# Hi-FT/ERD

Hardware: AMD Instinct MI355X
Metric: images/sec GFL-R50 40+40 incre step @1333x800 (higher is better)
Workload: dtype f32; 1 GPU; gfl_r50_fpn first_40_incre_last_40 ERD (BASELINE configs[1]), 1333x800 padded to 800x1344, fp32, procedural weights; batch_per_gpu=4, global_batch=4, parallelism=dp1

## Files before the change

### erd_amd/_lib.py

```python
from __future__ import annotations

import ctypes as C
import os

_HERE = os.path.dirname(os.path.abspath(__file__))
LIB_PATH = os.environ.get("ERD_HIP_LIB") or os.path.join(_HERE, "lib", "liberd_hip.so")

ERD_MAX_SEG = 5
ERD_MAX_TAPS = 9
ERD_SQNORM_PARTS = 1024

c_float_p = C.c_void_p
i64 = C.c_int64
i32 = C.c_int
f32 = C.c_float


class ConvSeg(C.Structure):
    _fields_ = [("inp", C.c_void_p), ("out", C.c_void_p), ("res", C.c_void_p), ("alpha", C.c_void_p),
                ("mask", C.c_void_p), ("N", i32), ("IH", i32), ("IW", i32), ("GH", i32), ("GW", i32), ("OH", i32), ("OW", i32),
                ("in_nstride", i64), ("out_nstride", i64), ("res_nstride", i64),
                ("tap0", i32), ("ntaps", i32), ("oy", i32), ("ox", i32)]


# ... 34 lines not shown


class Levels(C.Structure):
    _fields_ = [("nseg", i32), ("off", i64 * ERD_MAX_SEG), ("cnt", i64 * ERD_MAX_SEG)]


P = C.c_void_p
_SIGNATURES = {
    "erd_set_cu_reserve": [i32],
    "erd_usable_cus": [],
    "erd_conv_igemm": [C.POINTER(ConvDesc), P],
    "erd_conv_igemm_ws_bytes": [i32],
    "erd_to_bf16": [P, P, i64, P],
    "erd_split3": [P, P, i64, P],
    "erd_conv_thin_enable": [i32],
    "erd_conv_thin_ok": [C.POINTER(ConvDesc)],
    "erd_weight_transpose_x3": [P, P, P, i32, i32, i32, i32, P],
    "erd_wino_weights_elems": [i32, i32],
    "erd_wino_weights": [P, P, i32, i32, i32, P],
    "erd_wino_conv3x3": [P, i32, P, i32, i32, P, P, i32, P, i32, P, P],
    "erd_wino_weights_x3_elems": [i32, i32],
    "erd_wino_weights_x3": [P, P, i32, i32, i32, P],
    "erd_wino_conv3x3_x3": [P, i32, P, i32, i32, P, P, i32, P, i32, P, P],
    "erd_wino_x3_couts_per_item": [P, i32, i32],
    "erd_wino_conv3x3_x3_gn": [P, i32, P, i32, i32, P, P, i32, P, P, C.c_size_t, P],
    "erd_wino_gn_finalize": [P, i32, i32, P, P, f32, P],
    "erd_wino_x3_gn_ws_bytes": [P, i32, i32],
    "erd_conv_wgrad": [C.POINTER(WgradDesc), P],
    "erd_wgrad_row3_slices": [C.POINTER(WgradDesc)],
    "erd_wgrad_reduce": [P, i32, i32, i32, P, P, P, i32, P, P],
    "erd_wgrad_reduce_rows": [P, i32, i32, i32, i32, P, i32, P],
    "erd_weight_transpose": [P, P, P, i32, i32, i32, i32, P],
    "erd_weight_transpose_bf16": [P, P, P, i32, i32, i32, i32, P],
    "erd_stem_conv7x7_bn_relu": [P, P, P, P, P, i32, i32, i32, P],
    "erd_maxpool3x3s2": [P, P, i32, i32, i32, i32, i32, P],
    "erd_bn_fold": [P, P, P, P, f32, P, P, i64, P],
    "erd_bn_fold_batch": [P, i32, i32, P],
    "erd_weight_prep_blocks": [i32, i32, i32, i32],
    "erd_weight_prep_batch": [P, i32, i32, P],
    "erd_relu_bwd_colsum": [P, P, P, i64, i32, i64, i64, P, i32, i32, P],
    "erd_bn_dgamma": [P, P, i32, P, P, f32, P, P, i32, i32, P],
    "erd_gn_relu_fwd": [P, P, P, P, P, P, i32, i64, i32, i32, C.POINTER(Levels), f32, i32, P],
    "erd_gn_relu_apply": [P, P, P, P, P, i32, i64, i32, i32, C.POINTER(Levels), i32, P],
    "erd_gn_relu_bwd": [P, P, P, P, P, P, P, P, P, i32, i64, i32, i32, C.POINTER(Levels), i32, P],
    "erd_upsample2x_add": [P, P, i32, i32, i32, i32, i32, i32, i64, i64, i32, P],
    "erd_upsample2x_add_bwd": [P, P, i32, i32, i32, i32, i32, i32, i64, i64, i32, P],
# ... 90 lines not shown
```

### erd_amd/csrc/winograd.hip

```cpp
#include "erd_common.h"
#include <type_traits>
#include <stdlib.h>
#include <algorithm>

namespace {

typedef float f32x4 __attribute__((ext_vector_type(4)));
typedef unsigned int u32x4 __attribute__((ext_vector_type(4)));
constexpr unsigned OOBV = 0x80000000u;

__device__ __forceinline__ float4 buf_load16_s(__amdgpu_buffer_rsrc_t r, unsigned voff, unsigned soff) {
    const u32x4 v = __builtin_amdgcn_raw_buffer_load_b128(r, voff, soff, 0);
    return make_float4(__uint_as_float(v.x), __uint_as_float(v.y), __uint_as_float(v.z), __uint_as_float(v.w));
}

constexpr int KS = 16;
constexpr int BN = 64;
constexpr int BNP = 128;
constexpr int RCS = 6;
#ifndef ERD_WINO_NCH
#define ERD_WINO_NCH 4
#endif
constexpr int NCH = ERD_WINO_NCH;
constexpr int MAXPIX = 64 * NCH;
constexpr int RAW_LDS_F4 = MAXPIX * RCS;
constexpr int V_F4 = 16 * 32 * (KS / 4);
constexpr int MAXREG = 16;

__device__ __forceinline__ float4 f4add(float4 a, float4 b) { return make_float4(a.x + b.x, a.y + b.y, a.z + b.z, a.w + b.w); }
__device__ __forceinline__ float4 f4sub(float4 a, float4 b) { return make_float4(a.x - b.x, a.y - b.y, a.z - b.z, a.w - b.w); }
__device__ __forceinline__ int vswz2(int row, int c) { return c ^ ((0 - (row >> 2)) & 3); }

#ifdef ERD_WINO_TRACE
__device__ unsigned long long g_wino_trace[256 * 8];
__device__ unsigned long long g_wino_trace_p[256 * 16];
#define ERD_T0(v) const unsigned long long v = __builtin_amdgcn_s_memtime()
#define ERD_TACC(acc, v) acc += __builtin_amdgcn_s_memtime() - v
#else
#define ERD_T0(v)
#define ERD_TACC(acc, v)
#endif

__global__ __launch_bounds__(256) void wino_weight_kernel(const float* __restrict__ w, float* __restrict__ U, int Cout,
                                                           int Cin, int flip) {
    const int cop = (Cout + 15) / 16 * 16;
    const int64_t idx = blockIdx.x * 256ll + threadIdx.x;
    if (idx >= (int64_t)cop * Cin) return;
    const int co = (int)(idx / Cin), ci = (int)(idx % Cin);
    float g[3][3];
#pragma unroll
// ... 951 lines not shown
            };
            for (int g = 0;;) {
                if (g >= slices_total) break;
                iter(P0{}, P1{});
                if (++g >= slices_total) break;
                iter(P1{}, P0{});
                ++g;
            }
        };
        if (t_half == 0) run(std::integral_constant<int, 0>{});
        else run(std::integral_constant<int, 1>{});
#ifdef ERD_WINO_TRACE
        if (wave == 0 && lane == 0 && blockIdx.x < 256) {
            g_wino_trace[blockIdx.x * 8 + 4] = __builtin_amdgcn_s_memtime() - t_begin;
            g_wino_trace[blockIdx.x * 8 + 5] = t_bar;
            g_wino_trace[blockIdx.x * 8 + 6] = t_ent;
            g_wino_trace[blockIdx.x * 8 + 7] = t_wait;
        }
#endif
    }
}

constexpr int HPIX = 208;

__global__ __launch_bounds__(512, 2) void wino_x3p_kernel(const WinoDesc p) {
    extern __shared__ __attribute__((aligned(16))) char smem[];
    constexpr unsigned RAWB = HPIX * RCS * 16, VOFF = 2 * RAWB, VB = VX_B, XOFF = VOFF + 2 * VB;
    float* sh_ss = reinterpret_cast<float*>(smem + XOFF);
    int* sh_item = reinterpret_cast<int*>(sh_ss + 4 * 2 * BNP);
    float* sh_gn = reinterpret_cast<float*>(sh_item + 4);
    char* const sm = smem;

    const int tid = threadIdx.x;
    const int Cin = p.Cin;
    const int nks = Cin / KS;
    const int nitems = p.nitems;
    const int ncb32 = (p.Cout + 31) / 32;
    int cur_item = blockIdx.x;


    const int wave = __builtin_amdgcn_readfirstlane(tid >> 6), lane = tid & 63;
    const int item0 = blockIdx.x;
    if (item0 >= nitems) return;

    const int li = lane & 31, h = lane >> 5;
    const int ri = wave & 3, cp = wave >> 2;
    const int t_chunk = tid & 3, t_tile = (tid >> 2) & 31;
    const int t_row = __builtin_amdgcn_readfirstlane(tid >> 7);
    const int rowA = t_row == 0 ? 0 : (t_row == 2 ? 2 : 1), rowB = t_row == 2 ? 1 : (t_row == 3 ? 3 : 2);

    const __amdgpu_buffer_rsrc_t rs_U = __builtin_amdgcn_make_buffer_rsrc(
        const_cast<void*>(p.U3), 0, (int)((size_t)16 * 3 * ncb32 * nks * 1024), 0x00020000);
    const unsigned u_lane = (unsigned)lane * 16u;
    const unsigned per_xl_b = (unsigned)ncb32 * (unsigned)nks * 1024u;
    const unsigned pos0_b = (unsigned)(ri * 4 * 3) * per_xl_b;
    const unsigned cb_b = (unsigned)nks * 1024u;
    const unsigned v_lane = (unsigned)(ri * 4 * 3 * 1024 + h * 512 + ((li ^ (h * 8)) * 16));
    WinoItem cur = wino_decode<BNP>(p, item0);
    int k_item = 0;
    unsigned u_item = (unsigned)__builtin_amdgcn_readfirstlane(((cur.cout0 >> 5) + 2 * cp) * nks * 1024);
    f32x16 acc[8];
    u32x4 ub[4][3];
    bf16x8 vf[2][3];
    auto load_u = [&](const int u, const unsigned soff) {
#pragma unroll
        for (int l = 0; l < 3; ++l)
            ub[u & 3][l] = __builtin_amdgcn_raw_buffer_load_b128(rs_U, u_lane, pos0_b + (unsigned)((u >> 1) * 3 + l) * per_xl_b + soff + (u & 1) * cb_b, 0);
    };

    WinoItem la = cur;
    int la_ks = 0, k_la = 0;
    unsigned la_soff = 0;
    bool la_valid = true;
    unsigned roff[2];
    float4 rv[2];
    __amdgpu_buffer_rsrc_t rs_in = __builtin_amdgcn_make_buffer_rsrc(const_cast<float*>(p.seg[0].in), 0, 0, 0x00020000);
    unsigned rdA = 0, rdB = 0, nrdA = 0, nrdB = 0;
    int tr_left = 0;
    auto item_geometry = [&](const WinoItem& it, unsigned (&ro)[2], unsigned& gA, unsigned& gB, __amdgpu_buffer_rsrc_t& rs) {
        const WinoSeg& sg = p.seg[it.s];
        rs = __builtin_amdgcn_make_buffer_rsrc(const_cast<float*>(sg.in), 0, (int)((long long)sg.N * sg.in_nstride * 4), 0x00020000);
        const int lbw = it.lbw, bw = 1 << lbw, bh = 32 >> lbw;
        const int pc_n = 2 * bw + 2, npix = (2 * bh + 2) * pc_n;
        const int recip = (65536 + pc_n - 1) / pc_n;
        const unsigned base_n = (unsigned)(it.n * sg.in_nstride);
#pragma unroll
        for (int i = 0; i < 2; ++i) {
            const int idx = tid + 512 * i;
            const int chunk = idx & 3, pix = idx >> 2;
            const int pr = (pix * recip) >> 16, pc = pix - pr * pc_n;
            const int iy = it.y0 - 1 + pr, ix = it.x0 - 1 + pc;
            ro[i] = OOBV;
            if (pix < npix && (unsigned)iy < (unsigned)sg.H && (unsigned)ix < (unsigned)sg.W)
                ro[i] = (base_n + (unsigned)((iy * sg.W + ix) * Cin + chunk * 4)) * 4u;
        }
        const int t_ty = t_tile >> lbw, t_tx = t_tile & (bw - 1);
        gA = (unsigned)((((2 * t_ty + rowA) * pc_n + 2 * t_tx) * RCS + t_chunk) * 16);
        gB = (unsigned)((((2 * t_ty + rowB) * pc_n + 2 * t_tx) * RCS + t_chunk) * 16);
    };
    struct Pending { float sc, sh; int claim, k; };
    auto request_item_data = [&](Pending& pe) {
        if (tid < BNP) {
            const int co = la.cout0 + tid;
            pe.sc = (p.scale && co < p.Cout) ? p.scale[co] : 1.f;
            pe.sh = (p.shift && co < p.Cout) ? p.shift[co] : 0.f;
        }
        if (tid == BNP) pe.claim = wino_claim(p, k_la);
        pe.k = k_la;
    };
    auto flush_pending = [&](const Pending& pe) {
        if (pe.k >= 0) {
            if (tid < BNP) {
                float* ss = sh_ss + (pe.k & 3) * (2 * BNP);
                ss[tid] = pe.sc;
                ss[BNP + tid] = pe.sh;
            }
            if (tid == BNP) sh_item[(pe.k + 1) & 1] = pe.claim;
        }
    };
    auto issue_next = [&](float4* dst) {
        if (la_valid) {
#pragma unroll
            for (int i = 0; i < 2; ++i) dst[i] = buf_load16_s(rs_in, roff[i], la_soff);
            la_soff += KS * 4;
            ++la_ks;
        }
    };
    auto advance_item = [&](Pending& pe) {
        if (la_valid && la_ks == nks) {
            const int nx = __builtin_amdgcn_readfirstlane(sh_item[(k_la + 1) & 1]);
            if (nx < nitems) {
                la = wino_decode<BNP>(p, nx);
                item_geometry(la, roff, nrdA, nrdB, rs_in);
                la_ks = 0;
                la_soff = 0;
                ++k_la;
                request_item_data(pe);
            } else la_valid = false;
        }
    };
    const bool st1_ok = (tid >> 2) + 128 < HPIX;
    auto store_raw = [&](const float4* src, const unsigned par) {
        int t = tid;
        asm volatile("" : "+v"(t));
        const unsigned st_base = (unsigned)(((t >> 2) * RCS + (t & 3)) * 16);
        *reinterpret_cast<float4*>(sm + par * RAWB + st_base) = src[0];
        if (st1_ok) *reinterpret_cast<float4*>(sm + par * RAWB + st_base + 128 * RCS * 16) = src[1];
    };
    float4 pd[2][4];
    auto transform_read = [&](const unsigned rpar) {
        const char* rA = sm + rpar * RAWB + rdA;
        const char* rB = sm + rpar * RAWB + rdB;
#pragma unroll
        for (int c = 0; c < 4; ++c) {
            pd[0][c] = *reinterpret_cast<const float4*>(rA + c * (RCS * 16));
            pd[1][c] = *reinterpret_cast<const float4*>(rB + c * (RCS * 16));
        }
        if (--tr_left == 0) {
            rdA = nrdA;
            rdB = nrdB;
            tr_left = nks;
        }
    };
    auto v_write_base = [&]() -> unsigned {
        int t = tid;
        asm volatile("" : "+v"(t));
        const int c = t & 3, tl = (t >> 2) & 31;
        return VOFF + (unsigned)(t_row * 4 * 3072 + (c >> 1) * 512 + ((tl ^ ((c >> 1) * 8)) * 16) + (c & 1) * 8);
    };
    auto row_pass = [&](float4 (&R)[4]) __attribute__((always_inline)) {
        if (t_row == 1) {
#pragma unroll
            for (int c = 0; c < 4; ++c) R[c] = f4add(pd[0][c], pd[1][c]);
        } else {
#pragma unroll
            for (int c = 0; c < 4; ++c) R[c] = f4sub(pd[0][c], pd[1][c]);
        }
    };
    unsigned long long t_d1 = 0, t_d2 = 0, t_d3 = 0, t_out = 0; (void)t_d1; (void)t_d2; (void)t_d3; (void)t_out;
    auto data_phase = [&](const unsigned par, const unsigned u_tail) __attribute__((always_inline)) {
        const unsigned npar = par ^ 1u;
        ERD_T0(ta);
        transform_read(npar);
        __builtin_amdgcn_sched_barrier(0);
// ... 168 lines not shown
                        float* cpt = p.colsum + (p.colsum_copies > 1 ? (blockIdx.x & (p.colsum_copies - 1)) * p.Cout : 0) + co0;
                        atomicAdd(cpt + 0, cs[gq].x); atomicAdd(cpt + 1, cs[gq].y); atomicAdd(cpt + 2, cs[gq].z); atomicAdd(cpt + 3, cs[gq].w);
                    }
                }
            }
            __syncthreads();
        }
        if (p.gn_part && tid < 32) {
            const float t = ((sh_gn[tid] + sh_gn[32 + tid]) + sh_gn[64 + tid]) + sh_gn[96 + tid];
            p.gn_part[(int64_t)cur_item * 32 + tid] = t;
        }
    };

    {
        float4 rvb[2];
#pragma unroll
        for (int i = 0; i < 2; ++i) { rv[i] = make_float4(0.f, 0.f, 0.f, 0.f); rvb[i] = rv[i]; }
        item_geometry(la, roff, nrdA, nrdB, rs_in);
        Pending pe;
        pe.sc = 1.f; pe.sh = 0.f; pe.claim = 0; pe.k = -1;
        request_item_data(pe);
        rdA = nrdA;
        rdB = nrdB;
        tr_left = nks;
        flush_pending(pe);
        pe.k = -1;
        issue_next(rv);
        issue_next(rvb);
#pragma unroll
        for (int q = 0; q < 4; ++q) load_u(q, u_item);
        store_raw(rv, 0);
        __syncthreads();
        transform_read(0);
        float4 R[4];
        row_pass(R);
        char* v = sm + v_write_base();
        wino_put_limbs(v + 0 * 3072, f4sub(R[0], R[2]));
        wino_put_limbs(v + 1 * 3072, f4add(R[1], R[2]));
        wino_put_limbs(v + 2 * 3072, f4sub(R[2], R[1]));
        wino_put_limbs(v + 3 * 3072, f4sub(R[1], R[3]));
        store_raw(rvb, 1);
        issue_next(rv);
        __syncthreads();
    }

    unsigned long long t_bar = 0, t_m = 0, t_d = 0; (void)t_bar; (void)t_m; (void)t_d;
    ERD_T0(t_begin);
    int g = 0;
    for (;;) {
        const int nxt_item = __builtin_amdgcn_readfirstlane(sh_item[(k_item + 1) & 1]);
        const bool has_next = nxt_item < nitems;
        const WinoItem nxt = has_next ? wino_decode<BNP>(p, nxt_item) : cur;
        const unsigned u_next = (unsigned)__builtin_amdgcn_readfirstlane(((nxt.cout0 >> 5) + 2 * cp) * nks * 1024);
#pragma unroll
        for (int q = 0; q < 8; ++q)
#pragma unroll
            for (int r = 0; r < 16; ++r) acc[q][r] = 0.f;
        for (int ks = 0; ks < nks; ++ks, ++g) {
            const unsigned par = (unsigned)(g & 1);
            const bool last = ks + 1 == nks;
            const unsigned u_cur = (unsigned)__builtin_amdgcn_readfirstlane((int)(u_item + (unsigned)ks * 1024u));
            const unsigned u_reload = (unsigned)__builtin_amdgcn_readfirstlane(
                (int)(last ? u_next : u_item + (unsigned)(ks + 1) * 1024u));
            { ERD_T0(tm); matrix_phase(par, u_cur, u_reload); ERD_TACC(t_m, tm); }
            __builtin_amdgcn_sched_barrier(0);
            { ERD_T0(td); data_phase(par, u_reload); ERD_TACC(t_d, td); }
            { ERD_T0(tb); __syncthreads(); ERD_TACC(t_bar, tb); }
        }
        { ERD_T0(to); output_stage((unsigned)((g - 1) & 1)); ERD_TACC(t_out, to); }
        if (!has_next) {
#ifdef ERD_WINO_TRACE
            if ((wave & 3) == 0 && lane == 0 && blockIdx.x < 256) {
                unsigned long long* tr = g_wino_trace_p + blockIdx.x * 16 + (wave >> 2) * 8;
                tr[0] = __builtin_amdgcn_s_memtime() - t_begin;
                tr[1] = t_bar;
                tr[2] = t_m;
                tr[3] = t_d;
                tr[4] = t_d1;
                tr[5] = t_d2;
                tr[6] = t_d3;
                tr[7] = t_out;
            }
#endif
            if (tid == 0 && p.sched) wino_rearm(p);
            break;
        }
        cur = nxt;
        cur_item = nxt_item;
        u_item = u_next;
        ++k_item;
    }
}

__global__ __launch_bounds__(512) void wino_gn_finalize_kernel(const WinoDesc p, float* __restrict__ mean_rstd, float eps) {
    const int G = p.Cout >> 3;
    const int nb = blockIdx.x, s = blockIdx.y, n = blockIdx.z;
    if (n >= p.seg[s].N) return;
    const int q = threadIdx.x & 31, il = threadIdx.x >> 5;
    double acc = 0.0;
    for (int r = 0; r < p.nreg; ++r) {
        const WinoRegion& rg = p.reg[r];
        if (rg.seg != s) continue;
        const int per_img = rg.nby * rg.nbx;
        const int64_t it0 = (int64_t)nb * p.blocks_per_nb + rg.block0 + (int64_t)n * per_img;
        for (int b = il; b < per_img; b += 16) acc += (double)p.gn_part[(it0 + b) * 32 + q];
    }
    __shared__ double red[16][32];
    red[il][q] = acc;
    __syncthreads();
    if (threadIdx.x < 16) {
        const int gi = threadIdx.x;
        double s1 = 0.0, s2 = 0.0;
        for (int l = 0; l < 16; ++l) { s1 += red[l][2 * gi]; s2 += red[l][2 * gi + 1]; }
        const double m = (double)p.seg[s].H * p.seg[s].W * 8.0;
// ... 18 lines not shown

extern "C" int erd_wino_weights(const float* w_ohwi, float* U, int Cout, int Cin, int flip, erd_stream_t stream) {
    ERD_REQUIRE(w_ohwi && U && Cout > 0 && Cin > 0 && Cin % KS == 0, "wino_weights: Cin=%d must be a multiple of %d", Cin, KS);
    const int64_t n = (int64_t)((Cout + 15) / 16 * 16) * Cin;
    hipLaunchKernelGGL(wino_weight_kernel, dim3((unsigned)((n + 255) / 256)), dim3(256), 0, (hipStream_t)stream, w_ohwi, U,
                       Cout, Cin, flip);
    return erd::check_launch("wino_weights");
}

#ifdef ERD_WINO_TRACE
extern "C" int erd_wino_trace(unsigned long long* out) {
    (void)hipDeviceSynchronize();
    return (int)hipMemcpyFromSymbol(out, HIP_SYMBOL(g_wino_trace), sizeof(g_wino_trace));
}
extern "C" int erd_wino_trace_p(unsigned long long* out) {
    (void)hipDeviceSynchronize();
    return (int)hipMemcpyFromSymbol(out, HIP_SYMBOL(g_wino_trace_p), sizeof(g_wino_trace_p));
}
#endif

extern "C" size_t erd_wino_weights_elems(int Cout, int Cin) { return (size_t)16 * ((Cout + 15) / 16 * 16) * Cin; }

namespace {
int wino_plan(WinoDesc& d, const erd_conv_seg* segs, int nseg, bool x3, int Cout, int& ncu, bool& phased) {
    ERD_REQUIRE(segs && nseg >= 1 && nseg <= ERD_MAX_SEG, "wino: bad args");
    d.nseg = nseg;
    static const int shapes = getenv("ERD_WINO_SHAPES") ? atoi(getenv("ERD_WINO_SHAPES")) : 1;
    int blocks = 0, nreg = 0;
    auto add_region = [&](int s, int N, int ty0, int tx0, int nby, int nbx, int lbw, int ty1, int tx1) {
        if (nby <= 0 || nbx <= 0) return;
        WinoRegion& r = d.reg[nreg++];
        r.seg = s; r.ty0 = ty0; r.tx0 = tx0; r.nby = nby; r.nbx = nbx; r.lbw = lbw; r.ty1 = ty1; r.tx1 = tx1;
        r.block0 = blocks;
        blocks += N * nby * nbx;
    };
    for (int s = 0; s < nseg; ++s) {
        const erd_conv_seg& g = segs[s];
        ERD_REQUIRE(g.in && g.out && g.IH == g.OH && g.IW == g.OW, "wino: segment %d is not a stride-1 same-size map", s);
        ERD_REQUIRE((int64_t)g.N * g.in_nstride < (1ll << 29) && (int64_t)g.N * g.out_nstride < (1ll << 29),
                    "wino: segment %d too large (32-bit byte offsets)", s);
        WinoSeg& w = d.seg[s];
        w.in = g.in;
        w.out = g.out;
        w.res = g.res;
        w.mask = g.mask;
        ERD_REQUIRE(!g.alpha, "wino: per-level scalars are not supported");
        w.N = g.N;
// ... 14 lines not shown
            add_region(s, g.N, 4 * nby, 0, 1, (TW + bw - 1) / bw, bw == 16 ? 4 : 3, TH, TW);
        }
        const int cbw = TW - 8 * nbx;
        if (cbw > 0 && nby > 0) {
            const int bw = cbw <= 2 ? 2 : cbw <= 4 ? 4 : 8, bh = 32 / bw;
            add_region(s, g.N, 0, 8 * nbx, (4 * nby + bh - 1) / bh, 1, bw == 2 ? 1 : bw == 4 ? 2 : 3, 4 * nby, TW);
        }
    }
    d.nreg = nreg;
    d.blocks_per_nb = blocks;
    {
        int dev = 0;
        hipDeviceProp_t prop;
        static int cached = 0;
        if (cached == 0 && hipGetDevice(&dev) == hipSuccess && hipGetDeviceProperties(&prop, dev) == hipSuccess)
            cached = prop.multiProcessorCount;
        ncu = erd::usable_cus(cached > 0 ? cached : 256);
    }
    const char* const e_mode = getenv("ERD_WINO_P");
    const int p_mode = e_mode ? atoi(e_mode) : 1;
    const int64_t i64 = (int64_t)blocks * ((Cout + BN - 1) / BN), i128 = (int64_t)blocks * (Cout / BNP);
    phased = x3 && p_mode != 0 && Cout % BNP == 0 && blocks > 0 &&
             (p_mode >= 2 || 16 * ((i128 + ncu - 1) / ncu) <= 10 * ((i64 + ncu - 1) / ncu));
    return 0;
}

int wino_launch(const erd_conv_seg* segs, int nseg, const float* U, const void* U3, int Cin, int Cout, const float* scale,
                const float* shift, int relu, float* colsum, int colsum_copies, int* sched, hipStream_t stream,
                float* gn_part = nullptr, size_t gn_part_bytes = 0) {
    ERD_REQUIRE(segs && (U || U3) && nseg >= 1 && nseg <= ERD_MAX_SEG, "wino: bad args");
    ERD_REQUIRE(Cin % KS == 0 && Cin >= 4 * KS && Cout > 0, "wino: Cin=%d must be a multiple of %d and at least %d", Cin, KS, 4 * KS);
    WinoDesc d;
    d.U = U;
    d.U3 = U3;
    d.Cin = Cin;
    d.Cout = Cout;
    d.scale = scale;
    d.shift = shift;
    d.relu = relu;
    d.colsum = colsum;
    ERD_REQUIRE(colsum_copies >= 0 && (colsum_copies & (colsum_copies - 1)) == 0, "wino: colsum_copies must be a power of two");
    d.colsum_copies = colsum_copies;
    d.sched = sched;
    d.gn_part = gn_part;
    ERD_REQUIRE(!colsum || Cout % 4 == 0, "wino: colsum needs Cout %% 4 == 0");
    int ncu = 0;
    bool phased = false;
    if (const int rc = wino_plan(d, segs, nseg, U3 != nullptr, Cout, ncu, phased)) return rc;
    const int blocks = d.blocks_per_nb;
    if (blocks == 0) return 0;
    const int ncb = phased ? Cout / BNP : (Cout + BN - 1) / BN;
    d.nitems = blocks * ncb;
    static const int persist = getenv("ERD_WINO_PERSIST") ? atoi(getenv("ERD_WINO_PERSIST")) : 1;
    const int grid = persist ? (d.nitems < ncu ? d.nitems : ncu) : d.nitems;
    if (persist != 1) d.sched = nullptr;
    if (gn_part) {
        ERD_REQUIRE(Cout % 8 == 0, "wino: GroupNorm statistics need Cout %% 8 == 0");
        ERD_REQUIRE(phased && !colsum, "wino: the fused GroupNorm statistics need the 128-couts-per-item kernel (erd_wino_x3_couts_per_item) and no column sums");
        for (int q = 0; q < nseg; ++q) {
            ERD_REQUIRE(!segs[q].res && !segs[q].mask, "wino: the fused GroupNorm statistics serve plain convolutions (segment %d has a residual / mask)", q);
        }
        ERD_REQUIRE(gn_part_bytes >= (size_t)d.nitems * 32 * sizeof(float), "wino: GroupNorm partial-sum workspace too small (%zu bytes for %d items)",
                    gn_part_bytes, d.nitems);
    }
    if (phased) {
        const size_t lds = (size_t)2 * HPIX * RCS * 16 + 2 * VX_B + 4 * 2 * BNP * sizeof(float) + 16 + 4 * 16 * 2 * sizeof(float);
        static bool attrp_done = false;
        if (!attrp_done) {
            (void)hipFuncSetAttribute(reinterpret_cast<const void*>(wino_x3p_kernel), hipFuncAttributeMaxDynamicSharedMemorySize, (int)lds);
            attrp_done = true;
        }
        hipLaunchKernelGGL(wino_x3p_kernel, dim3((unsigned)grid), dim3(512), lds, stream, d);
        return erd::check_launch("wino_conv3x3_x3p");
    }
    if (U3) {
        const size_t lds = (size_t)2 * RAW_LDS_F4 * sizeof(float4) + 2 * VX_B + 4 * 2 * XCH_B + 64 + 2048 + 16;
        static bool attr3_done = false;
        if (!attr3_done) {
            (void)hipFuncSetAttribute(reinterpret_cast<const void*>(wino_x3_kernel), hipFuncAttributeMaxDynamicSharedMemorySize, (int)lds);
            attr3_done = true;
        }
        hipLaunchKernelGGL(wino_x3_kernel, dim3((unsigned)grid), dim3(512), lds, stream, d);
        return erd::check_launch("wino_conv3x3_x3");
    }
    const size_t lds = (size_t)2 * (RAW_LDS_F4 + V_F4) * sizeof(float4) + 2048 + 16;
    static bool attr_done = false;
    if (!attr_done) {
        (void)hipFuncSetAttribute(reinterpret_cast<const void*>(wino_conv_kernel), hipFuncAttributeMaxDynamicSharedMemorySize,
                                  (int)lds);
        attr_done = true;
    }
    hipLaunchKernelGGL(wino_conv_kernel, dim3((unsigned)grid), dim3(512), lds, stream, d);
    return erd::check_launch("wino_conv3x3");
}
// ... 9 lines not shown
extern "C" size_t erd_wino_weights_x3_elems(int Cout, int Cin) { return (size_t)16 * 3 * ((Cout + 31) / 32 * 32) * Cin; }

extern "C" int erd_wino_weights_x3(const float* w_ohwi, void* U3, int Cout, int Cin, int flip, erd_stream_t stream) {
    ERD_REQUIRE(w_ohwi && U3 && Cout > 0 && Cin > 0 && Cin % KS == 0, "wino_weights_x3: Cin=%d must be a multiple of %d", Cin, KS);
    const int64_t n = (int64_t)((Cout + 31) / 32 * 32) * Cin;
    hipLaunchKernelGGL(wino_weight_x3_kernel, dim3((unsigned)((n + 255) / 256)), dim3(256), 0, (hipStream_t)stream, w_ohwi,
                       reinterpret_cast<unsigned short*>(U3), Cout, Cin, flip);
    return erd::check_launch("wino_weights_x3");
}

extern "C" int erd_wino_x3_couts_per_item(const erd_conv_seg* segs, int nseg, int Cout) {
    WinoDesc d;
    int ncu = 0;
    bool phased = false;
    if (wino_plan(d, segs, nseg, true, Cout, ncu, phased)) return -1;
    return phased ? BNP : BN;
}

extern "C" int erd_wino_conv3x3_x3(const erd_conv_seg* segs, int nseg, const void* U3, int Cin, int Cout,
                                   const float* scale, const float* shift, int relu, float* colsum, int colsum_copies,
                                   int* sched, erd_stream_t stream) {
    ERD_REQUIRE(U3, "wino_x3: null U3");
    return wino_launch(segs, nseg, nullptr, U3, Cin, Cout, scale, shift, relu, colsum, colsum_copies, sched, (hipStream_t)stream);
}

extern "C" int erd_wino_conv3x3_x3_gn(const erd_conv_seg* segs, int nseg, const void* U3, int Cin, int Cout, const float* scale,
                                      const float* shift, int relu, int* sched, float* gn_part, size_t gn_part_bytes,
                                      erd_stream_t stream) {
    ERD_REQUIRE(U3 && gn_part, "wino_x3_gn: null U3 / gn_part");
    return wino_launch(segs, nseg, nullptr, U3, Cin, Cout, scale, shift, relu, nullptr, 0, sched, (hipStream_t)stream, gn_part, gn_part_bytes);
}

extern "C" int erd_wino_gn_finalize(const erd_conv_seg* segs, int nseg, int Cout, const float* gn_part, float* mean_rstd, float eps,
                                    erd_stream_t stream) {
    ERD_REQUIRE(segs && gn_part && mean_rstd && Cout % BNP == 0, "wino_gn_finalize: bad args");
    WinoDesc d;
    int ncu = 0, nmax = 0;
    bool phased = false;
    if (const int rc = wino_plan(d, segs, nseg, true, Cout, ncu, phased)) return rc;
    ERD_REQUIRE(phased, "wino_gn_finalize: these segments run on the 64-couts-per-item kernel (no partial sums exist)");
    d.Cout = Cout;
    d.gn_part = const_cast<float*>(gn_part);
    for (int q = 0; q < nseg; ++q) nmax = std::max(nmax, segs[q].N);
    hipLaunchKernelGGL(wino_gn_finalize_kernel, dim3((unsigned)(Cout / BNP), (unsigned)nseg, (unsigned)nmax), dim3(512), 0, (hipStream_t)stream, d,
                       mean_rstd, eps);
    return erd::check_launch("wino_gn_finalize");
// ... 10 lines not shown
```

### erd_amd/kernels.py

```python
from __future__ import annotations

import ctypes as C
import os as _os
from typing import Dict, List, Optional, Sequence, Tuple

import torch

from . import _lib
from ._lib import ConvDesc, Levels, WgradDesc, call

Tensor = torch.Tensor


_raw_stream = getattr(torch._C, "_cuda_getCurrentRawStream", None)


def _cur_stream() -> int:
    if _raw_stream is not None:
        return _raw_stream(torch.cuda.current_device())
    return torch.cuda.current_stream().cuda_stream


def _stream() -> C.c_void_p:
    return C.c_void_p(_cur_stream())
# ... 405 lines not shown
    if base is None or base.requires_grad:
        return wino_weights(w)
    x3 = wino_x3()
    ver = (w.data_ptr(), base._version, tuple(w.shape), x3)
    attr = "_erd_wino3" if x3 else "_erd_wino"
    hit = getattr(base, attr, None)
    if hit is None or hit[0] != ver:
        hit = (ver, wino_weights(w, x3=x3))
        setattr(base, attr, hit)
    return hit[1]


_WINO_SCHED = {}


def _wino_sched(device) -> Tensor:
    key = (str(device), _cur_stream())
    t = _WINO_SCHED.get(key)
    if t is None:
        t = _WINO_SCHED[key] = torch.zeros(2, dtype=torch.int32, device=device)
    return t


WINO_TRAIN_FWD = _os.environ.get("ERD_WINO_TRAIN_FWD", "1") != "0"
WINO_NOGRAD_FWD = _os.environ.get("ERD_WINO_NOGRAD_FWD", "1") != "0"
WINO_DGRAD = _os.environ.get("ERD_WINO_DGRAD", "1") != "0"
WINO_TEACHER = _os.environ.get("ERD_WINO_TEACHER", "1") != "0"
WINO_FROZEN_TRUNK = _os.environ.get("ERD_WINO_FROZEN_TRUNK", "0") == "1"
RECORDED = False


class distillation_forward:

    def __init__(self, winograd=None):
        self.winograd = WINO_FROZEN_TRUNK if winograd is None else winograd

    def __enter__(self):
        global WINO_NOGRAD_FWD
        self.keep = WINO_NOGRAD_FWD
        WINO_NOGRAD_FWD = self.winograd
        return self

    def __exit__(self, *exc):
        global WINO_NOGRAD_FWD
        WINO_NOGRAD_FWD = self.keep
        return False


def wino_ok(Cin: int, k: int, stride: int, pad: int) -> bool:
    return WINOGRAD and COMPUTE in ("f32", "f32x3") and k == 3 and stride == 1 and pad == 1 and Cin % 16 == 0 and Cin >= 64


def wino_conv3x3(xs: Sequence[Tensor], U: Tensor, outs: Sequence[Tensor], Cout: int, scale: Optional[Tensor] = None,
                 shift: Optional[Tensor] = None, relu: bool = False, res: Optional[Sequence[Optional[Tensor]]] = None,
                 mask: Optional[Sequence[Tensor]] = None, colsum: Optional[Tensor] = None, kname: str = "conv_wino_fwd") -> None:
    _require_gpu(U, *xs, *outs)
    from ._lib import ConvSeg
    segs = (ConvSeg * len(xs))()
    Cin = xs[0].shape[3]
    for i, (x, o) in enumerate(zip(xs, outs)):
        assert x.shape[:3] == o.shape[:3] and o.shape[3] == Cout and x.shape[3] == Cin
        assert x.dtype == torch.float32 and o.dtype == torch.float32, "the Winograd kernel is fp32 (maps and arithmetic)"
        _fill_seg(segs[i], x, o, x.shape[1], x.shape[2], None if res is None else res[i], None,
                  None if mask is None else mask[i])
    flop = 2.0 * sum(o.shape[0] * o.shape[1] * o.shape[2] for o in outs) * Cout * 9 * Cin
    nbytes = (4.0 * (sum(x.numel() for x in xs) + sum(o.numel() for o in outs)) + U.numel() * U.element_size()) if _TIMING is not None else 0.0
    if _TIMING is not None and U.dtype == torch.bfloat16 and int(_lib.load().erd_wino_x3_couts_per_item(segs, len(xs), Cout)) == 128:
        kname += "_p"
    _timed_call(kname, flop, "erd_wino_conv3x3_x3" if U.dtype == torch.bfloat16 else "erd_wino_conv3x3", segs, len(xs), _p(U), Cin, Cout, _p(scale), _p(shift),
                1 if relu else 0, _p(colsum), (colsum.numel() // Cout if colsum is not None else 0),
                _p(_wino_sched(U.device)), _stream(), nbytes=nbytes,
                tag=f"px{sum(o.shape[0] * o.shape[1] * o.shape[2] for o in outs)} {Cin}->{Cout} k3s1" if TIMING_DETAIL else "")


class _PrepRecipe:
    __slots__ = ("kind", "src", "rowscale", "out", "Cout", "ntaps", "Cin", "flip", "owner", "version", "level", "stamp",
                 "src_ptr", "rs_ptr")

    def matches(self, owner, src: Tensor, rowscale: Optional[Tensor]) -> bool:
        return (self.owner is owner and owner._version == self.version and src.data_ptr() == self.src_ptr and
                (0 if rowscale is None else rowscale.data_ptr()) == self.rs_ptr)


class ParamPrep:
    def __init__(self, device):
        self.device = torch.device(device)
        self.recipes: Dict[tuple, _PrepRecipe] = {}
        self.stamp = 0
        self._tables = None
        self._gtables: Dict[int, list] = {}
        self.group_of = None
        self.on_stale = None

    def _stale(self) -> None:
# ... 867 lines not shown
```

### include/erd_hip.h

```cpp
#ifndef ERD_HIP_H_
#define ERD_HIP_H_

#include <stddef.h>
#include <stdint.h>

#ifdef __cplusplus
extern "C" {
#endif

#define ERD_ABI_VERSION 6
#define ERD_MAX_SEG 5
#define ERD_MAX_TAPS 9

#define ERD_EINVAL (-1)
#define ERD_EUNSUPPORTED (-2)

typedef void* erd_stream_t;

enum { ERD_F32 = 0, ERD_BF16 = 1 };

int erd_abi_version(void);
int erd_set_cu_reserve(int n);
int erd_usable_cus(void);
int erd_probe_build(void);
// ... 31 lines not shown
    const void* w_x3;
} erd_conv_desc;

int erd_conv_igemm(const erd_conv_desc* d, erd_stream_t stream);
size_t erd_conv_igemm_ws_bytes(int max_tiles);
int erd_conv_thin_enable(int on);
int erd_conv_thin_ok(const erd_conv_desc* d);
int erd_to_bf16(const float* src, void* dst, int64_t n, erd_stream_t stream);
int erd_split3(const float* src, void* dst, int64_t n, erd_stream_t stream);

size_t erd_wino_weights_elems(int Cout, int Cin);
int erd_wino_weights(const float* w_ohwi, float* U, int Cout, int Cin, int flip ,
                     erd_stream_t stream);
int erd_wino_conv3x3(const erd_conv_seg* segs, int nseg, const float* U, int Cin, int Cout, const float* scale,
                     const float* shift, int relu, float* colsum, int colsum_copies ,
                     int* sched ,
                     erd_stream_t stream);

size_t erd_wino_weights_x3_elems(int Cout, int Cin);
int erd_wino_weights_x3(const float* w_ohwi, void* U3, int Cout, int Cin, int flip, erd_stream_t stream);
int erd_wino_conv3x3_x3(const erd_conv_seg* segs, int nseg, const void* U3, int Cin, int Cout, const float* scale,
                        const float* shift, int relu, float* colsum, int colsum_copies, int* sched, erd_stream_t stream);
int erd_wino_x3_couts_per_item(const erd_conv_seg* segs, int nseg, int Cout);
int erd_wino_conv3x3_x3_gn(const erd_conv_seg* segs, int nseg, const void* U3, int Cin, int Cout, const float* scale,
                           const float* shift, int relu, int* sched, float* gn_part, size_t gn_part_bytes, erd_stream_t stream);
int erd_wino_gn_finalize(const erd_conv_seg* segs, int nseg, int Cout, const float* gn_part, float* mean_rstd, float eps,
                         erd_stream_t stream);
size_t erd_wino_x3_gn_ws_bytes(const erd_conv_seg* segs, int nseg, int Cout);

typedef struct {
    int64_t x_off, dz_off;
    int N, IH, IW, GH, GW, OH, OW;
    int64_t x_nstride, dz_nstride;
} erd_wgrad_seg;

typedef struct {
    const float* x;
    const float* dz;
    int64_t x_elems, dz_elems;
    int nseg;
    erd_wgrad_seg seg[ERD_MAX_SEG];
    int Cin, Cout, ntaps;
    int dy[ERD_MAX_TAPS], dx[ERD_MAX_TAPS];
    int in_stride, out_stride, oy, ox;
    float* part;
    int nsplit;
// ... 205 lines not shown
```

Baseline: 121.5 images/sec.

## Split Winograd x3p work evenly across CUs with stream-K partial-sum handover

Adds a balanced variant of the persistent Winograd x3 kernel. It partitions the total item×K-slice work evenly over a grid sized to the CU count, instead of having blocks claim whole items dynamically. Items split between blocks write partial accumulators to a workspace slab, and the last contributor, found through an atomic ticket, reduces them and runs the output stage. This targets the tail imbalance when the item count does not divide evenly across CUs. In exchange it adds extra global traffic and synchronisation for split items, and it needs a new workspace buffer.

```diff
diff --git a/erd_amd/_lib.py b/erd_amd/_lib.py
--- a/erd_amd/_lib.py
+++ b/erd_amd/_lib.py
@@ -80,6 +80,7 @@
     "erd_wino_weights_x3_elems": [i32, i32],
     "erd_wino_weights_x3": [P, P, i32, i32, i32, P],
     "erd_wino_conv3x3_x3": [P, i32, P, i32, i32, P, P, i32, P, i32, P, P],
+    "erd_wino_conv3x3_x3_bal": [P, i32, P, i32, i32, P, P, i32, P, i32, P, P, C.c_size_t, P],
     "erd_wino_x3_couts_per_item": [P, i32, i32],
     "erd_wino_conv3x3_x3_gn": [P, i32, P, i32, i32, P, P, i32, P, P, C.c_size_t, P],
     "erd_wino_gn_finalize": [P, i32, i32, P, P, f32, P],
diff --git a/erd_amd/csrc/wino_partition.h b/erd_amd/csrc/wino_partition.h
--- /dev/null
+++ b/erd_amd/csrc/wino_partition.h
@@ -0,0 +1,13 @@
+#pragma once
+#if defined(__HIPCC__) || defined(__CUDACC__)
+#define ERD_WINO_HD __host__ __device__ inline
+#else
+#define ERD_WINO_HD inline
+#endif
+
+ERD_WINO_HD long long wino_part_begin(long long U, int G, int b) { return U * b / G; }
+ERD_WINO_HD int wino_part_owner(long long U, int G, long long u) { return (int)(((u + 1) * G - 1) / U); }
+ERD_WINO_HD int wino_part_first(long long U, int G, int nks, int item) { return wino_part_owner(U, G, (long long)item * nks); }
+ERD_WINO_HD int wino_part_last(long long U, int G, int nks, int item) { return wino_part_owner(U, G, (long long)(item + 1) * nks - 1); }
+ERD_WINO_HD int wino_part_slot(long long U, int G, int nks, int b, int item) { return item == (int)(wino_part_begin(U, G, b) / nks) ? 0 : 1; }
+ERD_WINO_HD long long wino_part_longest(long long U, int G) { return (U + G - 1) / G; }
diff --git a/erd_amd/csrc/winograd.hip b/erd_amd/csrc/winograd.hip
--- a/erd_amd/csrc/winograd.hip
+++ b/erd_amd/csrc/winograd.hip
@@ -1,4 +1,5 @@
 #include "erd_common.h"
+#include "wino_partition.h"
 #include <type_traits>
 #include <stdlib.h>
 #include <algorithm>
@@ -26,6 +27,7 @@
 constexpr int RAW_LDS_F4 = MAXPIX * RCS;
 constexpr int V_F4 = 16 * 32 * (KS / 4);
 constexpr int MAXREG = 16;
+constexpr int BAL_HANDOVER_SLICES = 20;
 
 __device__ __forceinline__ float4 f4add(float4 a, float4 b) { return make_float4(a.x + b.x, a.y + b.y, a.z + b.z, a.w + b.w); }
 __device__ __forceinline__ float4 f4sub(float4 a, float4 b) { return make_float4(a.x - b.x, a.y - b.y, a.z - b.z, a.w - b.w); }
@@ -1023,8 +1025,18 @@
 }
 
 constexpr int HPIX = 208;
-
-__global__ __launch_bounds__(512, 2) void wino_x3p_kernel(const WinoDesc p) {
+constexpr unsigned BAL_SLOT_B = 128u * 512u * 4u;
+static_assert(BAL_SLOT_B == ERD_WINO_BAL_SLOT_BYTES, "the header's workspace formula");
+constexpr size_t BAL_TICKET_B = ERD_WINO_BAL_TICKET_BYTES;
+
+struct WinoBalWs {
+    float* slabs;
+    int* tickets;
+    unsigned slab_bytes, ticket_bytes;
+};
+
+template <bool BAL>
+__device__ __forceinline__ void wino_x3p_body(const WinoDesc& p, const WinoBalWs& ws) {
     extern __shared__ __attribute__((aligned(16))) char smem[];
     constexpr unsigned RAWB = HPIX * RCS * 16, VOFF = 2 * RAWB, VB = VX_B, XOFF = VOFF + 2 * VB;
     float* sh_ss = reinterpret_cast<float*>(smem + XOFF);
@@ -1037,12 +1049,20 @@
     const int nks = Cin / KS;
     const int nitems = p.nitems;
     const int ncb32 = (p.Cout + 31) / 32;
-    int cur_item = blockIdx.x;
+    const long long bal_U = BAL ? (long long)nitems * nks : 0;
+    const int bal_G = BAL ? (int)gridDim.x : 1;
+    const int u_first = BAL ? (int)wino_part_begin(bal_U, bal_G, (int)blockIdx.x) : 0;
+    const int u_stop = BAL ? (int)wino_part_begin(bal_U, bal_G, (int)blockIdx.x + 1) : 0;
+    int cur_item = BAL ? u_first / nks : (int)blockIdx.x;
 
 
     const int wave = __builtin_amdgcn_readfirstlane(tid >> 6), lane = tid & 63;
-    const int item0 = blockIdx.x;
+    const int item0 = cur_item;
     if (item0 >= nitems) return;
+    if (BAL && u_first >= u_stop) return;
+    const int seg_ks0 = BAL ? u_first - item0 * nks : 0;
+    int seg_u = u_first, seg_len = BAL ? min(nks - seg_ks0, u_stop - u_first) : nks;
+    bool seg_whole = !BAL || (seg_ks0 == 0 && seg_len == nks);
 
     const int li = lane & 31, h = lane >> 5;
     const int ri = wave & 3, cp = wave >> 2;
@@ -1059,7 +1079,7 @@
     const unsigned v_lane = (unsigned)(ri * 4 * 3 * 1024 + h * 512 + ((li ^ (h * 8)) * 16));
     WinoItem cur = wino_decode<BNP>(p, item0);
     int k_item = 0;
-    unsigned u_item = (unsigned)__builtin_amdgcn_readfirstlane(((cur.cout0 >> 5) + 2 * cp) * nks * 1024);
+    unsigned u_item = (unsigned)__builtin_amdgcn_readfirstlane((((cur.cout0 >> 5) + 2 * cp) * nks + seg_ks0) * 1024);
     f32x16 acc[8];
     u32x4 ub[4][3];
     bf16x8 vf[2][3];
@@ -1071,8 +1091,9 @@
 
     WinoItem la = cur;
     int la_ks = 0, k_la = 0;
-    unsigned la_soff = 0;
+    unsigned la_soff = (unsigned)(seg_ks0 * KS * 4);
     bool la_valid = true;
+    int la_item = item0, la_len = seg_len, la_u_end = u_first + seg_len, ntr_len = seg_len;
     unsigned roff[2];
     float4 rv[2];
     __amdgpu_buffer_rsrc_t rs_in = __builtin_amdgcn_make_buffer_rsrc(const_cast<float*>(p.seg[0].in), 0, 0, 0x00020000);
@@ -1106,7 +1127,7 @@
             pe.sc = (p.scale && co < p.Cout) ? p.scale[co] : 1.f;
             pe.sh = (p.shift && co < p.Cout) ? p.shift[co] : 0.f;
         }
-        if (tid == BNP) pe.claim = wino_claim(p, k_la);
+        if constexpr (!BAL) { if (tid == BNP) pe.claim = wino_claim(p, k_la); }
         pe.k = k_la;
     };
     auto flush_pending = [&](const Pending& pe) {
@@ -1116,7 +1137,7 @@
                 ss[tid] = pe.sc;
                 ss[BNP + tid] = pe.sh;
             }
-            if (tid == BNP) sh_item[(pe.k + 1) & 1] = pe.claim;
+            if constexpr (!BAL) { if (tid == BNP) sh_item[(pe.k + 1) & 1] = pe.claim; }
         }
     };
     auto issue_next = [&](float4* dst) {
@@ -1128,6 +1149,23 @@
         }
     };
     auto advance_item = [&](Pending& pe) {
+        if constexpr (BAL) {
+            if (la_valid && la_ks == la_len) {
+                if (la_u_end < u_stop) {
+                    ++la_item;
+                    la = wino_decode<BNP>(p, la_item);
+                    item_geometry(la, roff, nrdA, nrdB, rs_in);
+                    la_ks = 0;
+                    la_soff = 0;
+                    la_len = min(nks, u_stop - la_u_end);
+                    la_u_end += la_len;
+                    ntr_len = la_len;
+                    ++k_la;
+                    request_item_data(pe);
+                } else la_valid = false;
+            }
+            return;
+        }
         if (la_valid && la_ks == nks) {
             const int nx = __builtin_amdgcn_readfirstlane(sh_item[(k_la + 1) & 1]);
             if (nx < nitems) {
@@ -1160,7 +1198,7 @@
         if (--tr_left == 0) {
             rdA = nrdA;
             rdB = nrdB;
-            tr_left = nks;
+            tr_left = BAL ? ntr_len : nks;
         }
     };
     auto v_write_base = [&]() -> unsigned {
@@ -1375,10 +1413,15 @@
         request_item_data(pe);
         rdA = nrdA;
         rdB = nrdB;
-        tr_left = nks;
+        tr_left = BAL ? seg_len : nks;
         flush_pending(pe);
         pe.k = -1;
         issue_next(rv);
+        if constexpr (BAL) {
+            advance_item(pe);
+            flush_pending(pe);
+            pe.k = -1;
+        }
         issue_next(rvb);
 #pragma unroll
         for (int q = 0; q < 4; ++q) load_u(q, u_item);
@@ -1393,6 +1436,10 @@
         wino_put_limbs(v + 2 * 3072, f4sub(R[2], R[1]));
         wino_put_limbs(v + 3 * 3072, f4sub(R[1], R[3]));
         store_raw(rvb, 1);
+        if constexpr (BAL) {
+            advance_item(pe);
+            flush_pending(pe);
+        }
         issue_next(rv);
         __syncthreads();
     }
@@ -1401,17 +1448,18 @@
     ERD_T0(t_begin);
     int g = 0;
     for (;;) {
-        const int nxt_item = __builtin_amdgcn_readfirstlane(sh_item[(k_item + 1) & 1]);
-        const bool has_next = nxt_item < nitems;
+        const int nxt_item = BAL ? cur_item + 1 : __builtin_amdgcn_readfirstlane(sh_item[(k_item + 1) & 1]);
+        const bool has_next = BAL ? seg_u + seg_len < u_stop : nxt_item < nitems;
         const WinoItem nxt = has_next ? wino_decode<BNP>(p, nxt_item) : cur;
         const unsigned u_next = (unsigned)__builtin_amdgcn_readfirstlane(((nxt.cout0 >> 5) + 2 * cp) * nks * 1024);
 #pragma unroll
         for (int q = 0; q < 8; ++q)
 #pragma unroll
             for (int r = 0; r < 16; ++r) acc[q][r] = 0.f;
-        for (int ks = 0; ks < nks; ++ks, ++g) {
+        const int nsl = BAL ? seg_len : nks;
+        for (int ks = 0; ks < nsl; ++ks, ++g) {
             const unsigned par = (unsigned)(g & 1);
-            const bool last = ks + 1 == nks;
+            const bool last = ks + 1 == nsl;
             const unsigned u_cur = (unsigned)__builtin_amdgcn_readfirstlane((int)(u_item + (unsigned)ks * 1024u));
             const unsigned u_reload = (unsigned)__builtin_amdgcn_readfirstlane(
                 (int)(last ? u_next : u_item + (unsigned)(ks + 1) * 1024u));
@@ -1420,7 +1468,57 @@
             { ERD_T0(td); data_phase(par, u_reload); ERD_TACC(t_d, td); }
             { ERD_T0(tb); __syncthreads(); ERD_TACC(t_bar, tb); }
         }
-        { ERD_T0(to); output_stage((unsigned)((g - 1) & 1)); ERD_TACC(t_out, to); }
+        bool finish = true;
+        if constexpr (BAL) {
+            if (!seg_whole) {
+                const int first_b = wino_part_first(bal_U, bal_G, nks, cur_item);
+                const int ncontrib = wino_part_last(bal_U, bal_G, nks, cur_item) - first_b + 1;
+                const __amdgpu_buffer_rsrc_t rs_slab = __builtin_amdgcn_make_buffer_rsrc(ws.slabs, 0, (int)ws.slab_bytes, 0x00020000);
+                const __amdgpu_buffer_rsrc_t rs_tk = __builtin_amdgcn_make_buffer_rsrc(ws.tickets, 0, (int)ws.ticket_bytes, 0x00020000);
+                int t = tid;
+                asm volatile("" : "+v"(t));
+                const unsigned t16 = (unsigned)t * 16u;
+                const unsigned my_off = (unsigned)(2 * (int)blockIdx.x + wino_part_slot(bal_U, bal_G, nks, (int)blockIdx.x, cur_item)) * BAL_SLOT_B + t16;
+#pragma unroll
+                for (int q = 0; q < 8; ++q)
+#pragma unroll
+                    for (int r = 0; r < 4; ++r) {
+                        u32x4 v;
+                        v.x = __float_as_uint(acc[q][4 * r]); v.y = __float_as_uint(acc[q][4 * r + 1]);
+                        v.z = __float_as_uint(acc[q][4 * r + 2]); v.w = __float_as_uint(acc[q][4 * r + 3]);
+                        __builtin_amdgcn_raw_buffer_store_b128(v, rs_slab, my_off + (unsigned)((q * 4 + r) * 512 * 16), 0, 16 );
+                    }
+                asm volatile("s_waitcnt vmcnt(0)" ::: "memory");
+                __syncthreads();
+                if (t == 0) sh_item[0] = __builtin_amdgcn_raw_ptr_buffer_atomic_add_i32(1, rs_tk, (unsigned)cur_item * 4u, 0, 0);
+                __syncthreads();
+                finish = __builtin_amdgcn_readfirstlane(sh_item[0]) == ncontrib - 1;
+                if (finish) {
+                    const bool pair = ncontrib == 2;
+                    if (!pair) {
+#pragma unroll
+                        for (int q = 0; q < 8; ++q)
+#pragma unroll
+                            for (int r = 0; r < 16; ++r) acc[q][r] = 0.f;
+                    }
+                    for (int c = 0; c < ncontrib; ++c) {
+                        const int bb = first_b + c;
+                        if (pair && bb == (int)blockIdx.x) continue;
+                        const unsigned so = (unsigned)(2 * bb + wino_part_slot(bal_U, bal_G, nks, bb, cur_item)) * BAL_SLOT_B + t16;
+#pragma unroll
+                        for (int q = 0; q < 8; ++q)
+#pragma unroll
+                            for (int r = 0; r < 4; ++r) {
+                                const u32x4 v = __builtin_amdgcn_raw_buffer_load_b128(rs_slab, so + (unsigned)((q * 4 + r) * 512 * 16), 0, 16 );
+                                acc[q][4 * r] += __uint_as_float(v.x); acc[q][4 * r + 1] += __uint_as_float(v.y);
+                                acc[q][4 * r + 2] += __uint_as_float(v.z); acc[q][4 * r + 3] += __uint_as_float(v.w);
+                            }
+                    }
+                    if (t == 0) __builtin_amdgcn_raw_buffer_store_b32(0u, rs_tk, (unsigned)cur_item * 4u, 0, 16 );
+                }
+            }
+        }
+        if (finish) { ERD_T0(to); output_stage((unsigned)((g - 1) & 1)); ERD_TACC(t_out, to); }
         if (!has_next) {
 #ifdef ERD_WINO_TRACE
             if ((wave & 3) == 0 && lane == 0 && blockIdx.x < 256) {
@@ -1442,7 +1540,19 @@
         cur_item = nxt_item;
         u_item = u_next;
         ++k_item;
+        if constexpr (BAL) {
+            seg_u += seg_len;
+            seg_len = min(nks, u_stop - seg_u);
+            seg_whole = seg_len == nks;
+        }
     }
+}
+
+__global__ __launch_bounds__(512, 2) void wino_x3p_kernel(const WinoDesc p) {
+    wino_x3p_body<false>(p, WinoBalWs{nullptr, nullptr, 0u, 0u});
+}
+__global__ __launch_bounds__(512, 2) void wino_x3pb_kernel(const WinoDesc p, const WinoBalWs ws) {
+    wino_x3p_body<true>(p, ws);
 }
 
 __global__ __launch_bounds__(512) void wino_gn_finalize_kernel(const WinoDesc p, float* __restrict__ mean_rstd, float eps) {
@@ -1507,7 +1617,8 @@
 extern "C" size_t erd_wino_weights_elems(int Cout, int Cin) { return (size_t)16 * ((Cout + 15) / 16 * 16) * Cin; }
 
 namespace {
-int wino_plan(WinoDesc& d, const erd_conv_seg* segs, int nseg, bool x3, int Cout, int& ncu, bool& phased) {
+int wino_plan(WinoDesc& d, const erd_conv_seg* segs, int nseg, bool x3, int Cout, int& ncu, bool& phased, int Cin = 0,
+              int* bal_grid = nullptr) {
     ERD_REQUIRE(segs && nseg >= 1 && nseg <= ERD_MAX_SEG, "wino: bad args");
     d.nseg = nseg;
     static const int shapes = getenv("ERD_WINO_SHAPES") ? atoi(getenv("ERD_WINO_SHAPES")) : 1;
@@ -1568,12 +1679,23 @@
     const int64_t i64 = (int64_t)blocks * ((Cout + BN - 1) / BN), i128 = (int64_t)blocks * (Cout / BNP);
     phased = x3 && p_mode != 0 && Cout % BNP == 0 && blocks > 0 &&
              (p_mode >= 2 || 16 * ((i128 + ncu - 1) / ncu) <= 10 * ((i64 + ncu - 1) / ncu));
+    if (bal_grid) {
+        *bal_grid = 0;
+        const char* const e_bal = getenv("ERD_WINO_BAL");
+        const int bal_mode = e_bal ? atoi(e_bal) : 1;
+        if (phased && p_mode == 1 && bal_mode != 0 && Cin >= 4 * KS) {
+            const int nks = Cin / KS;
+            const long long U = i128 * nks;
+            const int G = (int)std::min<long long>(ncu, U);
+            if (bal_mode >= 2 || wino_part_longest(U, G) + BAL_HANDOVER_SLICES <= (i128 + ncu - 1) / ncu * nks) *bal_grid = G;
+        }
+    }
     return 0;
 }
 
 int wino_launch(const erd_conv_seg* segs, int nseg, const float* U, const void* U3, int Cin, int Cout, const float* scale,
                 const float* shift, int relu, float* colsum, int colsum_copies, int* sched, hipStream_t stream,
-                float* gn_part = nullptr, size_t gn_part_bytes = 0) {
+                float* gn_part = nullptr, size_t gn_part_bytes = 0, void* bal_ws = nullptr, size_t bal_ws_bytes = 0) {
     ERD_REQUIRE(segs && (U || U3) && nseg >= 1 && nseg <= ERD_MAX_SEG, "wino: bad args");
     ERD_REQUIRE(Cin % KS == 0 && Cin >= 4 * KS && Cout > 0, "wino: Cin=%d must be a multiple of %d and at least %d", Cin, KS, 4 * KS);
     WinoDesc d;
@@ -1592,7 +1714,8 @@
     ERD_REQUIRE(!colsum || Cout % 4 == 0, "wino: colsum needs Cout %% 4 == 0");
     int ncu = 0;
     bool phased = false;
-    if (const int rc = wino_plan(d, segs, nseg, U3 != nullptr, Cout, ncu, phased)) return rc;
+    int bal_grid = 0;
+    if (const int rc = wino_plan(d, segs, nseg, U3 != nullptr, Cout, ncu, phased, Cin, &bal_grid)) return rc;
     const int blocks = d.blocks_per_nb;
     if (blocks == 0) return 0;
     const int ncb = phased ? Cout / BNP : (Cout + BN - 1) / BN;
@@ -1616,6 +1739,22 @@
             (void)hipFuncSetAttribute(reinterpret_cast<const void*>(wino_x3p_kernel), hipFuncAttributeMaxDynamicSharedMemorySize, (int)lds);
             attrp_done = true;
         }
+        if (bal_grid > 0 && !gn_part && persist == 1 && bal_ws && (size_t)d.nitems * sizeof(int) <= BAL_TICKET_B &&
+            bal_ws_bytes >= BAL_TICKET_B + (size_t)2 * bal_grid * BAL_SLOT_B) {
+            static bool attrb_done = false;
+            if (!attrb_done) {
+                (void)hipFuncSetAttribute(reinterpret_cast<const void*>(wino_x3pb_kernel), hipFuncAttributeMaxDynamicSharedMemorySize, (int)lds);
+                attrb_done = true;
+            }
+            WinoBalWs ws;
+            ws.tickets = reinterpret_cast<int*>(bal_ws);
+            ws.slabs = reinterpret_cast<float*>(reinterpret_cast<char*>(bal_ws) + BAL_TICKET_B);
+            ws.ticket_bytes = (unsigned)((size_t)d.nitems * sizeof(int));
+            ws.slab_bytes = (unsigned)((size_t)2 * bal_grid * BAL_SLOT_B);
+            d.sched = nullptr;
+            hipLaunchKernelGGL(wino_x3pb_kernel, dim3((unsigned)bal_grid), dim3(512), lds, stream, d, ws);
+            return erd::check_launch("wino_conv3x3_x3pb");
+        }
         hipLaunchKernelGGL(wino_x3p_kernel, dim3((unsigned)grid), dim3(512), lds, stream, d);
         return erd::check_launch("wino_conv3x3_x3p");
     }
@@ -1671,6 +1810,14 @@
                                    int* sched, erd_stream_t stream) {
     ERD_REQUIRE(U3, "wino_x3: null U3");
     return wino_launch(segs, nseg, nullptr, U3, Cin, Cout, scale, shift, relu, colsum, colsum_copies, sched, (hipStream_t)stream);
+}
+
+extern "C" int erd_wino_conv3x3_x3_bal(const erd_conv_seg* segs, int nseg, const void* U3, int Cin, int Cout, const float* scale,
+                                       const float* shift, int relu, float* colsum, int colsum_copies, int* sched, void* ws,
+                                       size_t ws_bytes, erd_stream_t stream) {
+    ERD_REQUIRE(U3, "wino_x3_bal: null U3");
+    return wino_launch(segs, nseg, nullptr, U3, Cin, Cout, scale, shift, relu, colsum, colsum_copies, sched, (hipStream_t)stream, nullptr, 0,
+                       ws, ws_bytes);
 }
 
 extern "C" int erd_wino_conv3x3_x3_gn(const erd_conv_seg* segs, int nseg, const void* U3, int Cin, int Cout, const float* scale,
diff --git a/erd_amd/kernels.py b/erd_amd/kernels.py
--- a/erd_amd/kernels.py
+++ b/erd_amd/kernels.py
@@ -451,6 +451,16 @@
     return t
 
 
+def _wino_bal_ws(device) -> Tuple[Tensor, int]:
+    key = ("wino_bal", str(device), _cur_stream())
+    ws = _WS.get(key)
+    if ws is None:
+        nbytes = (1 << 16) + 2 * torch.cuda.get_device_properties(device).multi_processor_count * (128 * 512 * 4)
+        ws = torch.zeros(nbytes, dtype=torch.uint8, device=device)
+        _ws_replace(key, ws)
+    return ws, ws.numel()
+
+
 WINO_TRAIN_FWD = _os.environ.get("ERD_WINO_TRAIN_FWD", "1") != "0"
 WINO_NOGRAD_FWD = _os.environ.get("ERD_WINO_NOGRAD_FWD", "1") != "0"
 WINO_DGRAD = _os.environ.get("ERD_WINO_DGRAD", "1") != "0"
@@ -496,9 +506,14 @@
     nbytes = (4.0 * (sum(x.numel() for x in xs) + sum(o.numel() for o in outs)) + U.numel() * U.element_size()) if _TIMING is not None else 0.0
     if _TIMING is not None and U.dtype == torch.bfloat16 and int(_lib.load().erd_wino_x3_couts_per_item(segs, len(xs), Cout)) == 128:
         kname += "_p"
-    _timed_call(kname, flop, "erd_wino_conv3x3_x3" if U.dtype == torch.bfloat16 else "erd_wino_conv3x3", segs, len(xs), _p(U), Cin, Cout, _p(scale), _p(shift),
+    if U.dtype == torch.bfloat16:
+        ws, ws_bytes = _wino_bal_ws(U.device)
+        tail = (_p(_wino_sched(U.device)), _p(ws), ws_bytes, _stream())
+    else:
+        tail = (_p(_wino_sched(U.device)), _stream())
+    _timed_call(kname, flop, "erd_wino_conv3x3_x3_bal" if U.dtype == torch.bfloat16 else "erd_wino_conv3x3", segs, len(xs), _p(U), Cin, Cout, _p(scale), _p(shift),
                 1 if relu else 0, _p(colsum), (colsum.numel() // Cout if colsum is not None else 0),
-                _p(_wino_sched(U.device)), _stream(), nbytes=nbytes,
+                *tail, nbytes=nbytes,
                 tag=f"px{sum(o.shape[0] * o.shape[1] * o.shape[2] for o in outs)} {Cin}->{Cout} k3s1" if TIMING_DETAIL else "")
 
 
diff --git a/include/erd_hip.h b/include/erd_hip.h
--- a/include/erd_hip.h
+++ b/include/erd_hip.h
@@ -77,6 +77,12 @@
 int erd_wino_conv3x3_x3(const erd_conv_seg* segs, int nseg, const void* U3, int Cin, int Cout, const float* scale,
                         const float* shift, int relu, float* colsum, int colsum_copies, int* sched, erd_stream_t stream);
 int erd_wino_x3_couts_per_item(const erd_conv_seg* segs, int nseg, int Cout);
+#define ERD_WINO_BAL_TICKET_BYTES ((size_t)1 << 16)
+#define ERD_WINO_BAL_SLOT_BYTES ((size_t)128 * 512 * 4)
+#define ERD_WINO_BAL_WS_BYTES(cus) (ERD_WINO_BAL_TICKET_BYTES + (size_t)2 * (size_t)(cus) * ERD_WINO_BAL_SLOT_BYTES)
+int erd_wino_conv3x3_x3_bal(const erd_conv_seg* segs, int nseg, const void* U3, int Cin, int Cout, const float* scale,
+                            const float* shift, int relu, float* colsum, int colsum_copies, int* sched, void* ws, size_t ws_bytes,
+                            erd_stream_t stream);
 int erd_wino_conv3x3_x3_gn(const erd_conv_seg* segs, int nseg, const void* U3, int Cin, int Cout, const float* scale,
                            const float* shift, int relu, int* sched, float* gn_part, size_t gn_part_bytes, erd_stream_t stream);
 int erd_wino_gn_finalize(const erd_conv_seg* segs, int nseg, int Cout, const float* gn_part, float* mean_rstd, float eps,
```

New measurement: 121.5 images/sec. No clear change (-0.1%).
